# vincenthz/eccoxide

Hardware: AMD Instinct MI355X
Metric: variable-base scalarmuls/sec (batch) per GPU + achieved HBM GB/s vs roofline (higher is better)
Workload: dtype u32

## Files before the change

### __graft_entry__.py

```python
import os
import subprocess
import sys
from concurrent.futures import ThreadPoolExecutor

ROOT = os.path.dirname(os.path.abspath(__file__))
if ROOT not in sys.path:
    sys.path.insert(0, ROOT)


def build() -> None:
    jobs = str(min(6, os.cpu_count() or 1))
    subprocess.check_call(["make", "-C", os.path.join(ROOT, "eccoxide_amd", "csrc"), "-j", jobs, "ARCH=gfx950"])
    subprocess.check_call(["make", "-C", os.path.join(ROOT, "oracle")])
    subprocess.check_call(["make", "-C", os.path.join(ROOT, "tests", "cpp")])
    test_libs = [
        "hip",
        "hip_p256k1",
        "hip_ed25519",
        "hip_merged",
        "hip_signed",
        "hip_lo32",
        "hip_ecdsa",
        "hip_ed25519_sign",
        "hip_ecdsa_sign",
        "hip_h2c",
        "hip_g2",
        "hip_h2c_g2",
        "hip_pairing",
        "hip_x448",
        "hip_jubjub",
        "hip_msm",
        "hip_sat",
    ]
    with ThreadPoolExecutor(max_workers=int(jobs)) as pool:
        list(pool.map(lambda d: subprocess.check_call(["make", "-C", os.path.join(ROOT, "tests", d)]), test_libs))
    import eccoxide_amd
    from eccoxide_amd import _lib

    lib = _lib.load()
    assert lib.eccx_field_bytes(eccoxide_amd.P256R1) == 32


def smoke() -> None:
    import eccoxide_amd as E
    from eccoxide_amd import workload as W
    from tests import oracle_lib

    ora = oracle_lib.load()
    with E.Engine(0) as eng:
        for curve, n in (("p256r1", 300), ("ed25519", 300)):
            ks = W.random_scalars(curve, n, seed=1).tobytes()
            want_b = ora.base(curve, ks, threads=4)
            got_b = eng.scalarmul_base(curve, ks)
            assert got_b[0] == want_b[0] and got_b[1] == want_b[1], f"{curve}: fixed-base mismatch vs oracle"
            pts = want_b[0]
            ks2 = W.random_scalars(curve, n, seed=2).tobytes()
            want_v = ora.var(curve, ks2, pts, threads=4)
            got_d = eng.scalarmul_var(curve, ks2, pts)
            assert got_d[0] == want_v[0] and got_d[1] == want_v[1], f"{curve}: variable-base mismatch vs oracle"
            got_v = eng.scalarmul_var(curve, ks2, pts, want_proj=True)
            assert got_v[0] == want_v[0] and got_v[1] == want_v[1], f"{curve}: mirror variable-base mismatch vs oracle"
            assert got_v[2] == want_v[2], f"{curve}: un-normalised coordinates differ from the reference algorithm"
            for kw in ({"ct_scan": True}, {"ct_gather": True}):
                got_c = eng.scalarmul_base(curve, ks, **kw)
                assert got_c[0] == want_b[0] and got_c[1] == want_b[1], f"{curve} {kw}: secret-scalar fixed base mismatch vs oracle"
            got_c = eng.scalarmul_var(curve, ks2, pts, ct_scan=True)
            assert got_c[0] == want_v[0] and got_c[1] == want_v[1], f"{curve}: secret-scalar variable base mismatch vs oracle"
            from oracle import ecc_ref as R

            inf = None if curve == "ed25519" else got_d[1]
            enc = eng.point_compress(curve, got_d[0], inf)
            assert enc == R.point_compress_bytes(curve, got_d[0], inf), f"{curve}: point encoding differs from the oracle"
            back = eng.point_decompress(curve, enc)
            assert back[0] == got_d[0] and back[1] == (bytes(n) if inf is None else inf), f"{curve}: decompress(compress(P)) != P"
        curve, n = "bls12_381_g1", 200
        pts = ora.base(curve, W.random_scalars(curve, n, seed=3).tobytes(), threads=4)[0]
        ks = W.random_scalars(curve, n, seed=4).tobytes()
        want = ora.var(curve, ks, pts, threads=4)
        for opts in ({}, {"assume_subgroup": True}, {"ct_scan": True}, {"ct_scan": True, "assume_subgroup": True}):
            got = eng.scalarmul_var(curve, ks, pts, **opts)
            assert got[0] == want[0] and got[1] == want[1], f"{curve} {opts}: variable-base mismatch vs oracle"
        from tests import ed25519_ref as ED

        seeds = bytes(range(32)) + bytes(range(32, 64)) + bytes(32)
        msgs = [b"", b"smoke", bytes(200)]
        pubs = eng.ed25519_public_key(seeds)
        assert pubs[:32] == ED.public_key(seeds[:32]), "ed25519: public key differs from the model"
        sigs = eng.ed25519_sign(msgs, seeds)
        assert sigs[64:128] == ED.sign(seeds[32:64], msgs[1]), "ed25519: signature differs from the model"
        assert eng.ed25519_sign(msgs, seeds, pubs) == sigs and eng.ed25519_sign(msgs, seeds, ct_gather=True) == sigs
        assert eng.ed25519_verify(msgs, sigs, pubs) == bytes([E.SIG_VALID]) * 3, "ed25519: own signatures do not verify"
        from tests import ecdsa_ref as EC, ecdsa_sign_ref as ES

        d, k, dig = bytes(range(1, 97)), bytes(range(101, 197)), bytes(range(7, 103))
        keys, kst = eng.ecdsa_public_key("p256r1", d)
        sigs, sst = eng.ecdsa_sign("p256r1", dig, d, k)
        assert (sigs[64:128], sst[1]) == ES.sign_record(EC.CURVES["p256r1"], dig[32:64], d[32:64], k[32:64]), "ecdsa: signature differs from the model"
        assert kst + sst == bytes([E.SIGN_OK]) * 6 and eng.ecdsa_verify("p256r1", dig, sigs, keys) == bytes([E.SIG_VALID]) * 3, "ecdsa: own signatures do not verify"
        from tests import h2c_ref as H2C

        hmsgs, tag = [b"", b"smoke", bytes(200)], b"QUUX-V01-CS02-with-BLS12381G1_XMD:SHA-256_SSWU_RO_"
        assert eng.hash_to_g1(hmsgs, tag) == H2C.hash_records(hmsgs, tag), "bls12_381_g1: hash_to_curve differs from the model"
        assert eng.hash_to_g1(hmsgs, tag, nonuniform=True) == H2C.hash_records(hmsgs, tag, True), \
            "bls12_381_g1: encode_to_curve differs from the model"
        from tests import g2_ref as G2

        n = 24
        rows = W.random_scalars("bls12_381_g2", 2 * n, seed=5)
        ks = [int.from_bytes(r.tobytes(), "big") for r in rows]
        off = G2.point_of_x((1, 2))
        bases = [G2.mul(k, G2.G) for k in ks[n:n + 4]] * (n // 4)
        bases[1], bases[2] = off, G2.add(G2.G, off)
        kb, pb = rows[:n].tobytes(), b"".join(G2.to_record(p)[0] for p in bases)
        want = [G2.to_record(G2.mul(k, p)) for k, p in zip(ks[:n], bases)]
        want = (b"".join(w[0] for w in want), bytes(w[1] for w in want))
        want_b = [G2.to_record(G2.mul(k, G2.G)) for k in ks[:n]]
        want_b = (b"".join(w[0] for w in want_b), bytes(w[1] for w in want_b))
        for ct in (False, True):
# ... 89 lines not shown
```

### eccoxide_amd/csrc/kernels_coz.hpp

```cpp
#pragma once
#include <type_traits>
#include "inv_gcd.hpp"
#include "kernels_ct.hpp"

namespace eccx {

struct NoGlv {
  static constexpr int K_BITS = 0;
};
struct PrimeOrderBases : NoGlv {};

template <class G>
ECCX_DEV void glv_split(uint32_t (&k1)[5], uint32_t (&k2)[5], const uint8_t* __restrict__ kb) {
  uint32_t k[8];
#pragma unroll
  for (int i = 0; i < 8; ++i) {
    const uint8_t* b = kb + 28 - 4 * i;
    k[i] = ((uint32_t)b[0] << 24) | ((uint32_t)b[1] << 16) | ((uint32_t)b[2] << 8) | (uint32_t)b[3];
  }
  uint32_t prod[13];
#pragma unroll
  for (int i = 0; i < 13; ++i) prod[i] = 0;
#pragma unroll
  for (int i = 0; i < 8; ++i) {
// ... 159 lines not shown
  s2 = h2[4] >> 31;
  uint32_t c_1 = s1, c_2 = s2;
#pragma unroll
  for (int i = 0; i < 5; ++i) {
    const uint64_t a = (uint64_t)(h1[i] ^ (0u - s1)) + c_1;
    k1[i] = (uint32_t)a;
    c_1 = (uint32_t)(a >> 32);
    const uint64_t b = (uint64_t)(h2[i] ^ (0u - s2)) + c_2;
    k2[i] = (uint32_t)b;
    c_2 = (uint32_t)(b >> 32);
  }
}


template <class CU>
constexpr int urowc_words() { return ((3 * CU::N + 3) / 4) * 4; }

template <class CU>
ECCX_DEV void u2_load(U<CU, 1, 3>& x, U<CU, 1, 3>& y, const uint32_t* __restrict__ row) {
  constexpr int N = CU::N;
  constexpr int W = ((2 * N + 3) / 4) * 4;
  uint32_t w[W];
  const uint4* src = reinterpret_cast<const uint4*>(row);
#pragma unroll
  for (int i = 0; i < W / 4; ++i) {
    const uint4 q = src[i];
    w[4 * i] = q.x; w[4 * i + 1] = q.y; w[4 * i + 2] = q.z; w[4 * i + 3] = q.w;
  }
#pragma unroll
  for (int i = 0; i < N; ++i) { x.v[i] = w[i]; y.v[i] = w[N + i]; }
}

template <class CU>
constexpr int urow2_words() { return ((2 * CU::N + 3) / 4) * 4; }
#ifndef ECCX_CT_VAR_PK
#define ECCX_CT_VAR_PK 0
#endif
template <class CU, bool TAGGED = false>
ECCX_DEV void u2_store(uint32_t* __restrict__ row, const U<CU, 1, 3>& x, const U<CU, 1, 3>& y) {
  constexpr int N = CU::N;
  constexpr int W = urow2_words<CU>();
  constexpr uint32_t T = TAGGED ? CT_F32_TAG : 0u;
  uint32_t w[W];
#pragma unroll
  for (int i = 0; i < W; ++i) w[i] = (i < N ? x.v[i] : (i < 2 * N ? y.v[i - N] : 0u)) | T;
  uint4* dst = reinterpret_cast<uint4*>(row);
#pragma unroll
  for (int i = 0; i < W / 4; ++i) dst[i] = make_uint4(w[4 * i], w[4 * i + 1], w[4 * i + 2], w[4 * i + 3]);
}

template <class CU>
ECCX_DEV void ujac_madd_signed(UJac<CU>& r, bool& h_zero, bool& r_zero, const UJac<CU>& p,
                          const U<CU, 1, 3>& x2, const U<CU, 1, 3>& y2, bool neg) {
  auto z1z1 = u_sqr(p.z);
  auto u2 = u_mul(x2, z1z1);
  auto t = u_mul(p.z, z1z1);
  U<CU, 2, 4> sy;
  u_select(sy, neg, u_neg(y2), u_as<2, 4>(y2));
  auto s2 = u_mul(u_reduce(sy), t);
  auto h = u_reduce(u_sub(u2, p.x));
  auto rr = u_reduce(u_sub(s2, p.y));
  h_zero = u_is_zero_mod_p(h);
  r_zero = u_is_zero_mod_p(rr);
  auto hh = u_sqr(h);
  auto hhh = u_mul(h, hh);
  auto v = u_mul(p.x, hh);
  auto r2 = u_sqr(rr);
  auto x3 = u_reduce(u_sub(u_sub(u_sub(r2, hhh), v), v));
  r.x = x3;
  if constexpr (CU::KIND == UK_MONT) {
    r.y = u_fit<1, 3>(u_mul_add(rr, u_sub(v, x3), u_neg(p.y), hhh));
  } else if constexpr (UB<CU>::SPARSE) {
    r.y = u_mul_sub(rr, u_sub(v, x3), p.y, hhh);
  } else if constexpr (UBS<CU>::DENSE) {
    r.y = u_mul_sub(rr, u_sdiff(v, x3), p.y, hhh);
  } else {
    auto y3a = u_mul(rr, u_sub(v, x3));
    auto y1h = u_mul(p.y, hhh);
    r.y = u_reduce(u_sub(y3a, y1h));
  }
  r.z = u_fit<UJac<CU>::ZK, UJac<CU>::ZV>(u_mul(p.z, h));
}

template <class CU>
ECCX_DEV void uzaddu(U<CU, 1, 3>& x1, U<CU, 1, 3>& y1, U<CU, 1, 3>& x2, U<CU, 1, 3>& y2, U<CU, 1, 3>& d_out, bool& d_zero) {
  const auto d = u_reduce(u_sub(x1, x2));
  d_zero = u_is_zero_mod_p(d);
  const auto c = u_sqr(d);
  const U<CU, 1, 3> w1 = u_fit<1, 3>(u_mul(x1, c));
  const auto w2 = u_mul(x2, c);
  const auto e = u_reduce(u_sub(y1, y2));
  const auto dd = u_sqr(e);
  const U<CU, 1, 3> a1 = u_fit<1, 3>(u_mul(y1, u_sub(w1, w2)));
  const auto x3 = u_reduce(u_sub(u_sub(dd, w1), w2));
  const auto y3m = u_mul(e, u_sub(w1, x3));
  x2 = x3;
  y2 = u_reduce(u_sub(y3m, a1));
  x1 = w1;
  y1 = a1;
  d_out = d;
}

template <class CU>
ECCX_DEV void ujac_madd_ct(UJac<CU>& r, bool& h_zero, bool& r_zero, const UJac<CU>& p, const U<CU, 1, 3>& x2,
                           const U<CU, 1, 3>& y2) {
  auto z1z1 = u_sqr(p.z);
  auto u2 = u_mul(x2, z1z1);
  auto t = u_mul(p.z, z1z1);
  auto s2 = u_mul(y2, t);
  auto h = u_reduce(u_sub(u2, p.x));
  auto rr = u_reduce(u_sub(s2, p.y));
  h_zero = u_is_zero_mod_p_ct(h);
  r_zero = u_is_zero_mod_p_ct(rr);
  auto hh = u_sqr(h);
  auto hhh = u_mul(h, hh);
  auto v = u_mul(p.x, hh);
  auto r2 = u_sqr(rr);
  auto x3 = u_reduce(u_sub(u_sub(u_sub(r2, hhh), v), v));
  r.x = x3;
  if constexpr (CU::KIND == UK_MONT) {
    r.y = u_fit<1, 3>(u_mul_add(rr, u_sub(v, x3), u_neg(p.y), hhh));
  } else if constexpr (UB<CU>::SPARSE) {
    r.y = u_mul_sub(rr, u_sub(v, x3), p.y, hhh);
  } else {
    auto y3a = u_mul(rr, u_sub(v, x3));
    auto y1h = u_mul(p.y, hhh);
    r.y = u_reduce(u_sub(y3a, y1h));
  }
  r.z = u_fit<UJac<CU>::ZK, UJac<CU>::ZV>(u_mul(p.z, h));
}

template <class CU>
ECCX_DEV void ujac_dbl_affine(U<CU, 1, 3>& x3, U<CU, 1, 3>& y3, U<CU, 1, 3>& z3, U<CU, 1, 3>& sv, U<CU, 1, 3>& y8v,
                              const U<CU, 1, 3>& px, const U<CU, 1, 3>& py) {
  const auto xx = u_sqr(px);
  const auto yy = u_sqr(py);
  const auto yyyy = u_sqr(yy);
  const auto xyy = u_mul(px, yy);
  const auto s2 = u_add(xyy, xyy);
  sv = u_reduce(u_add(s2, s2));
  const auto y4 = u_add(yyyy, yyyy);
  const auto y8 = u_add(y4, y4);
  y8v = u_reduce(u_add(y8, y8));
  if constexpr (CU::Sat::A0 == 1) {
    const auto m = u_reduce(u_add(u_add(xx, xx), xx));
    x3 = u_reduce(u_sub(u_sub(u_sqr(m), sv), sv));
    y3 = u_reduce(u_sub(u_mul(m, u_sub(sv, x3)), y8v));
  } else {
    U<CU, 1, 3> one;
#pragma unroll
    for (int i = 0; i < CU::N; ++i) one.v[i] = CU::ONE[i];
    const auto xm = u_sub(xx, one);
    const auto m = u_reduce(u_add(u_add(xm, xm), xm));
    x3 = u_reduce(u_sub(u_sub(u_sqr(m), sv), sv));
    y3 = u_reduce(u_sub(u_mul(m, u_sub(sv, x3)), y8v));
  }
  z3 = u_reduce(u_add(py, py));
}

template <class CU, int WB, bool ASSUME_PRIME = false>
constexpr int coz_full_windows() {
  using CS = typename CU::Sat;
  constexpr int NWIN = (8 * CS::SB + 1 + WB - 1) / WB;
  return (CS::PRIME_ORDER || ASSUME_PRIME) ? (8 * CS::SB - CS::NBITS + 1) / WB + 1 : NWIN;
}
#ifndef ECCX_CT_VAR_BITS
#define ECCX_CT_VAR_BITS 4
#endif

#ifndef ECCX_COZ_OCC_U14
#define ECCX_COZ_OCC_U14 3
#endif
#ifndef ECCX_COZ_OCC_BLS
#define ECCX_COZ_OCC_BLS 2
#endif
#ifndef ECCX_COZ_OCC_U9
#define ECCX_COZ_OCC_U9 4
#endif
#ifndef ECCX_COZ_NESTED_LADDER
#define ECCX_COZ_NESTED_LADDER 1
#endif
template <class CU, bool GLV>
constexpr int coz_occupancy() {
  return CU::N <= 9 ? ECCX_COZ_OCC_U9
                    : (CU::N <= 14 ? (GLV ? ECCX_OCC_U14 : (CU::KIND == UK_MONT ? ECCX_COZ_OCC_BLS : ECCX_COZ_OCC_U14)) : ECCX_OCC_U18);
}


template <class CU, class G, bool GLV, bool FUSED = false, int WB = 5, bool CT = false>
__global__ void __launch_bounds__(WG, (coz_occupancy<CU, GLV>())) k_scalarmul_coz_unsat(size_t n, const uint8_t* __restrict__ scalars,
                                                                                 const uint8_t* __restrict__ points,
                                                                                 uint32_t* __restrict__ rows_out,
                                                                                 uint8_t* __restrict__ flags,
                                                                                 uint32_t* __restrict__ scratch, uint32_t opts,
                                                                                 const uint8_t* __restrict__ base_scalars = nullptr,
                                                                                 const uint32_t* __restrict__ utable = nullptr) {
  static_assert(!(GLV && FUSED), "the verify shape takes any curve point");
  static_assert(!(CT && FUSED), "the verify shape has no secret-scalar form");
  constexpr bool ASSUME_PRIME = std::is_same<G, PrimeOrderBases>::value;
  constexpr bool LATTICE = GlvLattice<G>::value;
  static_assert(!(LATTICE && CT), "the secret-scalar endomorphism ladder is written for the unsigned split");
  static_assert(!ASSUME_PRIME || CT, "PrimeOrderBases only narrows the secret-scalar form's collision windows");
  static_assert(WB >= 3 && WB <= 5, "table rows 1 .. 2^(WB-1) must fit the slab");
  constexpr int TBL = 1 << (WB - 1);
  using CS = typename CU::Sat;
  constexpr bool ISO = CS::A0 == 1;
  constexpr int L = CS::L;
  constexpr int N = CU::N;
  constexpr int FB = CS::FB;
  constexpr int SB = CS::SB;
  static_assert(!GLV || SB == 32, "the split is written for 256-bit scalars");
  constexpr int NWIN = GLV ? (G::K_BITS + 1 + WB - 1) / WB : (8 * SB + 1 + WB - 1) / WB;
  constexpr int S = (!GLV && !CT) ? (8 * SB + 1) % WB : 0;
  constexpr int NWIN_MAIN = S != 0 ? (8 * SB + 1) / WB : NWIN;
  constexpr bool SHARED_INV = !ISO && !CT;
  static_assert(WG == 256, "the shared inversion multiplies the values of four waves");
  constexpr int WR = urowc_words<CU>();
  static_assert(!ISO || WR >= 16 + N, "row 0 holds the split scalar and zeta");
  using T = U<CU, 1, 3>;
  uint32_t* slab = scratch + ((size_t)blockIdx.x * FAST_TABLE_ROWS * WG + threadIdx.x) * (size_t)WR;
  auto row = [&](uint32_t e) { return slab + (size_t)e * WG * WR; };
  constexpr int WC = urow2_words<CU>();
  static_assert(!CT || (size_t)TBL * WC <= (size_t)(FAST_TABLE_ROWS - 1 - TBL) * WR, "the compact table must fit the free rows");
  uint32_t* cslab = scratch + ((size_t)blockIdx.x * FAST_TABLE_ROWS + (TBL + 1)) * WG * (size_t)WR + (size_t)threadIdx.x * WC;
  auto crow = [&](uint32_t e) { return cslab + (size_t)(e - 1) * WG * WC; };
  uint32_t iter = 0u;
  for (size_t base = (size_t)blockIdx.x * WG; base < n; base += (size_t)gridDim.x * WG, ++iter) {
    const size_t gid = base + threadIdx.x;
    const bool active = gid < n;
    const size_t idx = active ? gid : n - 1;
    const uint8_t* __restrict__ k = scalars + idx * (size_t)SB;
    if constexpr (GLV) {
      uint32_t k1[5], k2[5], s1 = 0, s2 = 0;
      if constexpr (LATTICE) glv_split_lattice<G>(k1, k2, s1, s2, k);
      else glv_split<G>(k1, k2, k);
      uint4* d = reinterpret_cast<uint4*>(row(0));
      d[0] = make_uint4(k1[0], k1[1], k1[2], k1[3]);
      d[1] = make_uint4(k1[4], s1, 0u, 0u);
      d[2] = make_uint4(k2[0], k2[1], k2[2], k2[3]);
      d[3] = make_uint4(k2[4], s2, 0u, 0u);
    }
    const uint32_t* kw = row(0);

    T one;
#pragma unroll
    for (int i = 0; i < N; ++i) one.v[i] = CU::ONE[i];
    UJac<CU> q;
    bool rejected = false;
    {
      Fe<L> rx, ry;
      fe_load_be<CS>(rx, points + idx * (size_t)(2 * FB));
      fe_load_be<CS>(ry, points + idx * (size_t)(2 * FB) + FB);
      if (opts & OPT_VALIDATE) {
        Fe<L> mx, my;
        fe_to_mont<CS>(mx, rx);
        fe_to_mont<CS>(my, ry);
        rejected = !(fe_is_canonical<CS>(rx) && fe_is_canonical<CS>(ry) && on_curve<CS>(mx, my));
      }
      q.x = u_as<1, 3>(u_to_mont<CU>(rx));
      q.y = u_as<1, 3>(u_to_mont<CU>(ry));
    }
    if constexpr (FUSED) {
      if (opts & OPT_NEGATE_B) q.y = u_reduce(u_neg(q.y));
    }
    q.z = u_as<UJac<CU>::ZK, UJac<CU>::ZV>(one);
    u3_store<CU>(row(1), q.x, q.y, one);

    auto booth = [&](int w, bool second, uint32_t& d, bool& neg) {
      uint32_t w6;
      if constexpr (GLV) {
        const uint32_t* h = kw + (second ? 8 : 0);
        const int pos = WB * w - 1 + 32;
        const int wi = pos >> 5, sh = pos & 31;
        const uint32_t lo = (wi >= 1 && wi <= 5) ? h[wi - 1] : 0u;
        const uint32_t hi = (wi <= 4) ? h[wi] : 0u;
        w6 = (uint32_t)((((uint64_t)hi << 32) | lo) >> sh) & ((1u << (WB + 1)) - 1u);
        const uint32_t s = ~((w6 >> WB) - 1u);
        const uint32_t m = (((1u << (WB + 1)) - w6 - 1u) & s) | (w6 & ~s);
        d = (m >> 1) + (m & 1u);
        neg = (s & 1u) != 0;
        if constexpr (LATTICE) neg = neg != (h[5] != 0u);
      } else if constexpr (S != 0) {
        booth_digit_aligned<WB, SB, S>(k, w, d, neg);
      } else {
        booth_digit<WB, SB>(k, w, d, neg);
      }
    };

    bool degenerate = false;
    {
      T px = q.x, py = q.y;
      T tx, ty, ratio;
      T zacc = one;
      {
        T x3, y3, sv, y8v;
        ujac_dbl_affine<CU>(x3, y3, ratio, sv, y8v, px, py);
        degenerate = u_is_zero_mod_p(ratio);
        tx = x3;
        ty = y3;
        px = sv;
        py = y8v;
        if constexpr (!ISO) zacc = ratio;
        u3_store<CU>(row(2), tx, ty, ratio);
      }
      for (int d = 3; d <= TBL; ++d) {
        bool dz;
        uzaddu<CU>(px, py, tx, ty, ratio, dz);
        degenerate = degenerate || dz;
        if constexpr (!ISO) zacc = u_fit<1, 3>(u_mul(zacc, ratio));
        u3_store<CU>(row(d), tx, ty, ratio);
      }
      T lam = one, next = ratio;
      if constexpr (ISO) {
        if constexpr (CT) u2_store<CU, (ECCX_CT_VAR_PK != 0)>(crow(TBL), tx, ty);
        else if constexpr (GLV) u3_store<CU>(row(TBL), tx, ty, u_fit<1, 3>(u_mul_k<CU>(tx, CU::BETA)));
      } else {
        if constexpr (SHARED_INV) {
          __shared__ uint32_t zsh[N][WG];
          const uint32_t tid = threadIdx.x;
          T zs;
          u_select(zs, degenerate, one, zacc);
#pragma unroll
          for (int i = 0; i < N; ++i) zsh[i][tid] = zs.v[i];
          __syncthreads();
          if ((uint32_t)__builtin_amdgcn_readfirstlane((int)(tid >> 6)) == (iter & 3u)) {
            const uint32_t col = tid & 63u;
            auto get = [&](int j) {
              T a;
#pragma unroll
              for (int i = 0; i < N; ++i) a.v[i] = zsh[i][col + 64u * j];
              return a;
            };
            auto put = [&](int j, const T& a) {
#pragma unroll
              for (int i = 0; i < N; ++i) zsh[i][col + 64u * j] = a.v[i];
            };
            const T p1 = u_fit<1, 3>(u_mul(get(0), get(1)));
            const T p2 = u_fit<1, 3>(u_mul(p1, get(2)));
            Fe<L> c;
            u_to_canonical<CU>(c, u_mul(p2, get(3)));
            fe_inv_gcd<CS>(c, c);
            T inv = u_as<1, 3>(u_to_mont<CU>(c));
            {
              const T a3 = get(3);
              put(3, u_fit<1, 3>(u_mul(inv, p2)));
              inv = u_fit<1, 3>(u_mul(inv, a3));
            }
            {
              const T a2 = get(2);
              put(2, u_fit<1, 3>(u_mul(inv, p1)));
              inv = u_fit<1, 3>(u_mul(inv, a2));
            }
            const T a0 = get(0), a1 = get(1);
            put(0, u_fit<1, 3>(u_mul(inv, a1)));
            put(1, u_fit<1, 3>(u_mul(inv, a0)));
          }
          __syncthreads();
#pragma unroll
          for (int i = 0; i < N; ++i) lam.v[i] = zsh[i][tid];
          __syncthreads();
        } else {
          Fe<L> c;
          u_to_canonical<CU>(c, zacc);
          fe_inv_gcd<CS>(c, c);
          lam = u_as<1, 3>(u_to_mont<CU>(c));
        }
        const T l2 = u_fit<1, 3>(u_sqr(lam));
        const T l3 = u_fit<1, 3>(u_mul(l2, lam));
        const T xt = u_fit<1, 3>(u_mul(tx, l2)), yt = u_fit<1, 3>(u_mul(ty, l3));
        if constexpr (CT) u2_store<CU, (ECCX_CT_VAR_PK != 0)>(crow(TBL), xt, yt);
        else u3_store<CU>(row(TBL), xt, yt, one);
      }
      for (int d = TBL - 1; d >= 1; --d) {
        lam = u_fit<1, 3>(u_mul(lam, next));
        T x, y;
        u3_load<CU>(x, y, next, row(d));
        const T l2 = u_fit<1, 3>(u_sqr(lam));
        const T l3 = u_fit<1, 3>(u_mul(l2, lam));
        const T xs = u_fit<1, 3>(u_mul(x, l2));
        const T ys = u_fit<1, 3>(u_mul(y, l3));
        if constexpr (CT) u2_store<CU, (ECCX_CT_VAR_PK != 0)>(crow(d), xs, ys);
        else if constexpr (GLV) u3_store<CU>(row(d), xs, ys, u_fit<1, 3>(u_mul_k<CU>(xs, CU::BETA)));
        else u3_store<CU>(row(d), xs, ys, one);
      }
      if constexpr (ISO) {
        uint32_t* zdst = row(0) + 16;
#pragma unroll
        for (int i = 0; i < N; ++i) zdst[i] = lam.v[i];
      }
    }

    if constexpr (CT) {
      constexpr int FULLW = GLV ? 1 : coz_full_windows<CU, WB, ASSUME_PRIME>();
      constexpr int HALVES = GLV ? 2 : 1;
      auto lookup = [&](int w, bool second, T& ex, T& ey, uint32_t& d) {
        bool neg;
        booth(w, second, d, neg);
        neg = neg != second;
#if ECCX_CT_VAR_PK
        {
          uint64_t acc[N];
#pragma unroll
          for (int p = 0; p < N; ++p) acc[p] = 0;
#pragma unroll 2
          for (int j = 1; j <= TBL; ++j) {
            uint32_t m;
            asm("v_cndmask_b32_e64 %0, 0, 1.0, %1" : "=v"(m) : "s"(__builtin_amdgcn_uicmp(d, (uint32_t)j, 32 )));
            const uint64_t m2 = m;
            const uint4* src = reinterpret_cast<const uint4*>(crow(j));
            uint4 v[WC / 4];
#pragma unroll
            for (int c = 0; c < WC / 4; ++c) v[c] = src[c];
#pragma unroll
            for (int p = 0; p < N; ++p) {
              const uint4 qv = v[p / 2];
              ct_fsel2(acc[p], (p & 1) ? (((uint64_t)qv.w << 32) | qv.z) : (((uint64_t)qv.y << 32) | qv.x), m2);
            }
          }
#pragma unroll
          for (int i = 0; i < N; ++i) {
            ex.v[i] = (uint32_t)(acc[i / 2] >> (32 * (i & 1))) & ~CT_F32_TAG;
            ey.v[i] = (uint32_t)(acc[(N + i) / 2] >> (32 * ((N + i) & 1))) & ~CT_F32_TAG;
          }
        }
#else
        u_set_zero(ex);
        u_set_zero(ey);
#pragma unroll 2
        for (int j = 1; j <= TBL; ++j) {
          T cx, cy;
          u2_load<CU>(cx, cy, crow(j));
          const uint64_t m = __builtin_amdgcn_uicmp(d, (uint32_t)j, 32 );
          u_cmov_ct(ex, m, cx);
          u_cmov_ct(ey, m, cy);
        }
#endif
        if constexpr (GLV) {
          if (second) ex = u_fit<1, 3>(u_mul_k<CU>(ex, CU::BETA));
        }
        U<CU, 2, 4> sy;
        u_select_ct(sy, neg, u_neg(ey), u_as<2, 4>(ey));
        ey = u_reduce(sy);
      };
      T zero;
      u_set_zero(zero);
      using TZ = U<CU, UJac<CU>::ZK, UJac<CU>::ZV>;
      {
        T ex, ey;
        uint32_t d;
        lookup(NWIN - 1, false, ex, ey, d);
        q.x = ex;
        q.y = ey;
        u_select_ct(q.z, d == 0, u_as<UJac<CU>::ZK, UJac<CU>::ZV>(zero), u_as<UJac<CU>::ZK, UJac<CU>::ZV>(one));
      }
#pragma unroll 1
      for (int win = NWIN - 1; win >= 0; --win) {
        if (win != NWIN - 1) {
#pragma unroll 1
          for (int j = 0; j < WB; ++j) {
            UJac<CU> t;
            ujac_dbl<CU>(t, q);
            q = t;
          }
        }
#pragma unroll 1
        for (int half = (win == NWIN - 1) ? 1 : 0; half < HALVES; ++half) {
          T ex, ey;
          uint32_t d;
          lookup(win, half != 0, ex, ey, d);
          const bool q_inf = u_limbs_all_zero(q.z);
          const bool e_skip = d == 0;
          UJac<CU> sum;
          bool hz, rz;
          ujac_madd_ct<CU>(sum, hz, rz, q, ex, ey);
          if (win < FULLW) {
            T dx, dy, dz, sv, y8v;
            ujac_dbl_affine<CU>(dx, dy, dz, sv, y8v, ex, ey);
            const bool same_x = hz & !q_inf & !e_skip;
            const uint64_t mt = ct_mask(same_x & rz);
            const uint64_t mc = ct_mask(same_x & !rz);
            u_cmov_ct(sum.x, mt, dx);
            u_cmov_ct(sum.y, mt, dy);
            u_cmov_ct(sum.z, mt, TZ(u_as<UJac<CU>::ZK, UJac<CU>::ZV>(dz)));
            u_cmov_ct(sum.z, mc, TZ(u_as<UJac<CU>::ZK, UJac<CU>::ZV>(zero)));
          }
          const uint64_t mi = ct_mask(q_inf), mk = ct_mask(!e_skip);
          u_cmov_ct(sum.x, mi, ex);
          u_cmov_ct(sum.y, mi, ey);
          u_cmov_ct(sum.z, mi, TZ(u_as<UJac<CU>::ZK, UJac<CU>::ZV>(one)));
          u_cmov_ct(q.x, mk, sum.x);
          u_cmov_ct(q.y, mk, sum.y);
          u_cmov_ct(q.z, mk, sum.z);
        }
      }
    } else {
      constexpr int WIN_END = S != 0 ? -1 : 0;
      {
        uint32_t d;
        bool neg;
        booth(NWIN_MAIN - 1, false, d, neg);
        T tx, ty;
        u2_load<CU>(tx, ty, row(d ? d : 1));
        U<CU, 2, 4> sy;
        u_select(sy, neg, u_neg(ty), u_as<2, 4>(ty));
        q.x = tx;
        q.y = u_reduce(sy);
        q.z = u_as<UJac<CU>::ZK, UJac<CU>::ZV>(one);
        if (d == 0) u_set_zero(q.z);
      }
      bool fix_lane = false;
      auto dbl_step = [&](bool fix) __attribute__((always_inline)) {
        UJac<CU> t;
        if constexpr (UBS<CU>::DENSE) {
          ujac_dbl_merged<CU>(t, q);
          if (fix) {
            const uint64_t keep = ct_mask(!fix_lane);
            u_cmov_ct(t.x, keep, q.x);
            u_cmov_ct(t.y, keep, q.y);
            u_cmov_ct(t.z, keep, q.z);
          }
          q = t;
        } else {
          ujac_dbl<CU>(t, q);
          if (fix) {
            u_select(q.x, fix_lane, t.x, q.x);
            u_select(q.y, fix_lane, t.y, q.y);
            u_select(q.z, fix_lane, t.z, q.z);
          } else {
            q = t;
          }
        }
      };
      auto add_step = [&](int win, bool second) __attribute__((always_inline)) -> bool {
        uint32_t d;
        bool neg;
        booth(win, second, d, neg);
        if (second && !LATTICE) neg = !neg;
        T ex, ey;
        if constexpr (GLV) {
          T eb;
          u3_load<CU>(ex, ey, eb, row(d ? d : 1));
          if (second) ex = eb;
        } else {
          u2_load<CU>(ex, ey, row(d ? d : 1));
        }
        const bool q_inf = u_limbs_all_zero(q.z);
        const bool e_skip = (d == 0);
        UJac<CU> sum;
        bool hz, rz;
        ujac_madd_signed<CU>(sum, hz, rz, q, ex, ey, neg);
        const bool same_x = hz && !q_inf && !e_skip;
        fix_lane = same_x && rz;
        if (same_x && !rz) u_set_zero(sum.z);
        if (__builtin_amdgcn_ballot_w64(q_inf) != 0) {
          U<CU, 2, 4> sy;
          u_select(sy, neg, u_neg(ey), u_as<2, 4>(ey));
          u_select(sum.x, q_inf, ex, sum.x);
          u_select(sum.y, q_inf, u_reduce(sy), sum.y);
          u_select(sum.z, q_inf, u_as<UJac<CU>::ZK, UJac<CU>::ZV>(one), sum.z);
        }
        const bool keep = e_skip || fix_lane;
        u_select(q.x, keep, q.x, sum.x);
        u_select(q.y, keep, q.y, sum.y);
        u_select(q.z, keep, q.z, sum.z);
        return __builtin_amdgcn_ballot_w64(fix_lane) != 0;
      };
      if constexpr (!GLV && ECCX_COZ_NESTED_LADDER) {
#pragma unroll 1
        for (int win = NWIN_MAIN - 2; win >= WIN_END; --win) {
          const int nd = (S != 0 && win < 0) ? S : WB;
#pragma unroll 1
          for (int sub = 0; sub < nd; ++sub) dbl_step(false);
          if (add_step(win, false)) dbl_step(true);
        }
      } else {
        int win, sub;
        if constexpr (GLV) {
          win = NWIN_MAIN - 1;
          sub = WB + 1;
        } else {
          win = NWIN_MAIN - 2;
          sub = 0;
        }
        bool fix_pending = false;
        while (win >= WIN_END) {
          const int nd = (S != 0 && win < 0) ? S : WB;
          bool step_done;
          if (fix_pending || sub < nd) {
            dbl_step(fix_pending);
            fix_pending = false;
            step_done = true;
          } else {
            fix_pending = add_step(win, GLV && sub == WB + 1);
            step_done = !fix_pending;
          }
          if (step_done) {
            if (sub < nd + (GLV ? 1 : 0)) {
              ++sub;
            } else {
              sub = 0;
              --win;
            }
          }
        }
      }
    }
    if constexpr (ISO) {
      T zeta;
      const uint32_t* zsrc = row(0) + 16;
#pragma unroll
      for (int i = 0; i < N; ++i) zeta.v[i] = zsrc[i];
      q.z = u_fit<UJac<CU>::ZK, UJac<CU>::ZV>(u_mul(q.z, zeta));
    }
    if constexpr (FUSED) ucomb_accumulate<CU, false>(q, base_scalars + idx * (size_t)SB, utable);
    if (active) {
      u3_store<CU>(rows_out + idx * (size_t)urow3_words<CU>(), q.x, q.y, u_fit<1, 3>(q.z));
      flags[idx] = rejected ? 2 : (degenerate ? FLAG_REDO : 0);
    }
  }
}

}
```

### eccoxide_amd/csrc/ufe.hpp

```cpp
#pragma once
#include "fe.hpp"

#include <type_traits>

#ifndef ECCX_SOLINAS_REDUCE
#define ECCX_SOLINAS_REDUCE 1
#endif

namespace eccx {

#include "umad_chunks.inc"

__device__ __forceinline__ void smad1_k(uint64_t& acc, uint32_t a, int32_t k) {
  asm("v_mad_i64_i32 %0, vcc, %1, %2, %0" : "+v"(acc) : "v"(a), "s"(k) : "vcc");
}

__device__ __forceinline__ void smad1_v(uint64_t& acc, int32_t a, int32_t b) {
  asm("v_mad_i64_i32 %0, vcc, %1, %2, %0" : "+v"(acc) : "v"(a), "v"(b) : "vcc");
}

template <int S>
__device__ __forceinline__ void ucarry_hi(uint64_t& acc) {
  uint64_t r;
  asm("v_mad_u64_u32 %0, vcc, %1, %2, 0" : "=&v"(r) : "v"((uint32_t)(acc >> 32)), "n"(1 << S) : "vcc");
// ... 789 lines not shown
  u_mul2_core_mont<C>(r.v, a.v, b.v, c.v, d.v);
  return r;
}

template <class C>
struct UBS {
  static constexpr bool OK = UB<C>::SPARSE || C::KIND == UK_MONT;
  static constexpr bool DENSE = C::KIND == UK_MONT_PP1 && !UB<C>::SPARSE;
  static constexpr int KKS = (int)((~(uint64_t)0 >> 1) / ((uint64_t)C::N * UB<C>::COL)) - 1;
  static_assert(!DENSE || (uint64_t)C::N * KKS * UB<C>::COL <= (~(uint64_t)0 >> 1) - 0xffffffffull * UB<C>::pp1_sum() -
                                                                ((uint64_t)1 << C::B) - ((uint64_t)1 << (63 - C::B)),
                "32-bit Montgomery digits overflow the signed columns");
  static constexpr bool ks_ok(int k) { return ((uint64_t)(k + 1) << C::B) <= ((uint64_t)1 << 31); }
};

template <class C, int K1, int V1, int K2, int V2, int K3, int V3, int K4, int V4>
ECCX_DEV auto u_mul_sub(const U<C, K1, V1>& a, const U<C, K2, V2>& b, const U<C, K3, V3>& c, const U<C, K4, V4>& d) {
  static_assert(UBS<C>::OK || UBS<C>::DENSE, "implemented for the Montgomery fields with room for signed columns");
  static_assert(K1 * K2 <= UBS<C>::KKS && K3 * K4 <= UBS<C>::KKS, "a product overflows the signed columns");
  static_assert(UBS<C>::ks_ok(K3) && UBS<C>::ks_ok(K4), "negated / signed operands must stay below 2^31");
  static_assert((uint32_t)(V1 * V2) < C::RP && (uint32_t)(V3 * V4) < C::RP, "result outside (0, 3p)");
  U<C, 1, 3> r;
  if constexpr (UB<C>::SPARSE) u_mul_sub_core_sparse<C, false>(r.v, a.v, b.v, c.v, d.v);
  else if constexpr (UBS<C>::DENSE) u_mul_sub_core_pp1<C, false>(r.v, a.v, b.v, c.v, d.v);
  else u_mul_sub_core_mont<C, false>(r.v, a.v, b.v, c.v, d.v);
  return r;
}
template <class C, int K1, int V1, int K2, int V2, int K3, int V3>
ECCX_DEV auto u_mul_sub_2sqr(const U<C, K1, V1>& a, const U<C, K2, V2>& b, const U<C, K3, V3>& c) {
  static_assert(UBS<C>::OK || UBS<C>::DENSE, "implemented for the Montgomery fields with room for signed columns");
  static_assert(K1 * K2 <= UBS<C>::KKS && 2 * K3 * K3 <= UBS<C>::KKS, "a product overflows the signed columns");
  static_assert(UBS<C>::ks_ok(2 * K3), "doubled / negated operands must stay below 2^31");
  static_assert((uint32_t)(V1 * V2) < C::RP && (uint32_t)(2 * V3 * V3) < C::RP, "result outside (0, 3p)");
  U<C, 1, 3> r;
  if constexpr (UB<C>::SPARSE) u_mul_sub_core_sparse<C, true>(r.v, a.v, b.v, c.v, c.v);
  else if constexpr (UBS<C>::DENSE) u_mul_sub_core_pp1<C, true>(r.v, a.v, b.v, c.v, c.v);
  else u_mul_sub_core_mont<C, true>(r.v, a.v, b.v, c.v, c.v);
  return r;
}

template <class C, int K, int V>
struct US {
  static_assert(K >= 1 && UBS<C>::ks_ok(K), "signed limbs must stay below 2^31");
  static_assert(V >= 1 && V <= 4096, "value bound out of range");
  int32_t v[C::N];
};

template <class C, int V1, int V2>
ECCX_DEV auto u_sdiff(const U<C, 1, V1>& a, const U<C, 1, V2>& b) {
  US<C, 1, (V1 > V2 ? V1 : V2)> r;
#pragma unroll
  for (int i = 0; i < C::N; ++i) r.v[i] = (int32_t)(a.v[i] - b.v[i]);
  return r;
}

template <class C>
constexpr bool ubs_neg_side_ok(int kk) {
  return (uint64_t)C::N * (uint64_t)kk * UB<C>::COL <= (~(uint64_t)0 >> 1) - ((uint64_t)1 << (64 - C::B));
}

template <class C, int K1, int V1, int K2, int V2, int K3, int V3, int K4, int V4>
ECCX_DEV auto u_mul_sub(const U<C, K1, V1>& a, const US<C, K2, V2>& b, const U<C, K3, V3>& c, const U<C, K4, V4>& d) {
  static_assert(UBS<C>::DENSE, "signed operands are implemented for p = -1 mod 2^B with p + 1 as plain digits");
  static_assert(K1 * K2 <= UBS<C>::KKS && K3 * K4 <= UBS<C>::KKS, "a product overflows the signed columns");
  static_assert(UBS<C>::ks_ok(K1) && UBS<C>::ks_ok(K3) && UBS<C>::ks_ok(K4), "negated / signed operands must stay below 2^31");
  static_assert(ubs_neg_side_ok<C>(K1 * K2 + K3 * K4), "the negative side of a column overflows");
  static_assert((uint32_t)(V1 * V2 + V3 * V4) < C::RP, "result outside (0, 3p)");
  U<C, 1, 3> r;
  u_mul_sub_core_pp1<C, false, int32_t>(r.v, a.v, b.v, c.v, d.v);
  return r;
}
template <class C, int K1, int V1, int K2, int V2, int K3, int V3>
ECCX_DEV auto u_mul_sub_2sqr(const U<C, K1, V1>& a, const US<C, K2, V2>& b, const U<C, K3, V3>& c) {
  static_assert(UBS<C>::DENSE, "signed operands are implemented for p = -1 mod 2^B with p + 1 as plain digits");
  static_assert(K1 * K2 <= UBS<C>::KKS && 2 * K3 * K3 <= UBS<C>::KKS, "a product overflows the signed columns");
  static_assert(UBS<C>::ks_ok(K1) && UBS<C>::ks_ok(2 * K3), "doubled / negated operands must stay below 2^31");
  static_assert(ubs_neg_side_ok<C>(K1 * K2 + 2 * K3 * K3), "the negative side of a column overflows");
  static_assert((uint32_t)(V1 * V2 + 2 * V3 * V3) < C::RP, "result outside (0, 3p)");
  U<C, 1, 3> r;
  u_mul_sub_core_pp1<C, true, int32_t>(r.v, a.v, b.v, c.v, c.v);
  return r;
}

template <class C, int V1>
ECCX_DEV auto u_sqr2(const U<C, 1, V1>& a) {
  static_assert(UBS<C>::DENSE && UB<C>::LO32, "written for p = -1 mod 2^B with p + 1 as plain digits");
  static_assert(UB<C>::kk_ok(2, 1), "columns: a square with doubled terms carries a product with K1*K2 = 2");
  static_assert(UB<C>::KMAX >= 2, "limbs: the doubled operand a << 1 (below 2 * 2^B) stays below 2^32");
  static_assert(UB<C>::vout(2 * V1, V1) <= 3, "result too large: reduce the operand first");
  U<C, 1, UB<C>::vout(2 * V1, V1)> r;
  u_mul_core_mont<C, true, false, true, true>(r.v, a.v, a.v);
  return r;
}

template <class C, int K1, int V1>
ECCX_DEV auto u_sqr(const U<C, K1, V1>& a) {
  if constexpr (!UB<C>::ksq_ok(K1) || (UB<C>::vout(V1, V1) > 3)) {
    return u_sqr(u_reduce(a));
  } else {
    U<C, 1, UB<C>::vout(V1, V1)> r;
    u_mul_core<C, true, false>(r.v, a.v, a.v);
    return r;
  }
}

template <class C, int K1, int V1>
ECCX_DEV auto u_mul_k(const U<C, K1, V1>& a, const uint32_t (&k)[C::N]) {
  if constexpr (!UB<C>::kk_ok(K1, 1) || (UB<C>::vout(V1, 1) > 3)) {
    return u_mul_k(u_reduce(a), k);
  } else {
    U<C, 1, UB<C>::vout(V1, 1)> r;
    u_mul_core<C, false, true>(r.v, a.v, k);
    return r;
  }
}

template <class C>
ECCX_DEV U<C, 1, 2> u_mul_k_exit(const U<C, 1, 3>& a, const uint32_t (&k)[C::N]) {
  static_assert(UB<C>::MONT && UB<C>::vout(3, 1) <= 2, "Montgomery fields; a reduced operand times a constant below p");
  U<C, 1, 2> r;
  u_mul_core_mont<C, false, true, false>(r.v, a.v, k);
  return r;
}

template <class C, int K1, int V1>
ECCX_DEV U<C, 1, 2> u_mul_small(const U<C, K1, V1>& a, uint32_t k) {
  static_assert(C::KIND == UK_PM19 || C::KIND == UK_GOLDILOCKS, "written for 2^255 - 19 and 2^448 - 2^224 - 1");
  constexpr int N = C::N;
  uint32_t t[N];
  uint64_t acc = 0;
#pragma unroll
  for (int i = 0; i < N; ++i) {
    umad1_v(acc, a.v[i], k);
    t[i] = (uint32_t)acc & C::MASK;
    acc >>= C::B;
  }
  if constexpr (C::KIND == UK_GOLDILOCKS) u_gold_tail<C>(t, acc);
  else u_pm_tail<C>(t, acc);
  U<C, 1, 2> r;
#pragma unroll
  for (int i = 0; i < N; ++i) r.v[i] = t[i];
  return r;
}

template <class C, int K1, int V1, int K2, int V2>
ECCX_DEV auto u_add(const U<C, K1, V1>& a, const U<C, K2, V2>& b) {
  if constexpr (K1 + K2 > UB<C>::KMAX) {
    if constexpr (K1 >= K2) return u_add(u_reduce(a), b);
    else return u_add(a, u_reduce(b));
  } else {
    U<C, K1 + K2, V1 + V2> r;
#pragma unroll
    for (int i = 0; i < C::N; ++i) r.v[i] = a.v[i] + b.v[i];
    return r;
  }
}

template <class C, int K1, int V1, int K2, int V2>
ECCX_DEV auto u_sub(const U<C, K1, V1>& a, const U<C, K2, V2>& b) {
  if constexpr (K2 != 1 || V2 > 3) {
    return u_sub(a, u_reduce(b));
  } else if constexpr (K1 + 2 > UB<C>::KMAX) {
    return u_sub(u_reduce(a), b);
  } else {
    U<C, K1 + 2, V1 + 4> r;
#pragma unroll
// ... 179 lines not shown
```

Measured before the change: 79.09 million.

## Use signed-difference madd and precomputed negated-y table entries in COZ ladder

For public-scalar, non-GLV curves with dense p = -1 mod 2^B, the mixed add now forms H and R as signed differences. It squares and multiplies them with new signed Montgomery kernels, which skips the reductions, and does the zero tests only on wave-uniform rare paths through Z3. The precomputed table also stores -y in its third slot, so the Booth digit sign picks a column at load time instead of negating and reducing each step. A signed co-Z addition for table building is added but left off by default, and a standalone signed-square check build is added to the setup.

```diff
diff --git a/__graft_entry__.py b/__graft_entry__.py
--- a/__graft_entry__.py
+++ b/__graft_entry__.py
@@ -32,8 +32,10 @@
         "hip_msm",
         "hip_sat",
     ]
+    makes = [["make", "-C", os.path.join(ROOT, "tests", d)] for d in test_libs]
+    makes.append(["make", "-C", os.path.join(ROOT, "tests", "hip"), "-f", "signed_sq_check.mk"])
     with ThreadPoolExecutor(max_workers=int(jobs)) as pool:
-        list(pool.map(lambda d: subprocess.check_call(["make", "-C", os.path.join(ROOT, "tests", d)]), test_libs))
+        list(pool.map(subprocess.check_call, makes))
     import eccoxide_amd
     from eccoxide_amd import _lib
 
diff --git a/eccoxide_amd/csrc/kernels_coz.hpp b/eccoxide_amd/csrc/kernels_coz.hpp
--- a/eccoxide_amd/csrc/kernels_coz.hpp
+++ b/eccoxide_amd/csrc/kernels_coz.hpp
@@ -265,6 +265,76 @@
   r.z = u_fit<UJac<CU>::ZK, UJac<CU>::ZV>(u_mul(p.z, h));
 }
 
+#ifndef ECCX_COZ_MADD_SIGNED_HR
+#define ECCX_COZ_MADD_SIGNED_HR 1
+#endif
+#ifndef ECCX_COZ_TABLE_NEG_Y
+#define ECCX_COZ_TABLE_NEG_Y 1
+#endif
+#ifndef ECCX_COZ_ZADDU_SIGNED
+#define ECCX_COZ_ZADDU_SIGNED 0
+#endif
+
+template <class CU>
+ECCX_DEV void u2_load_xc(U<CU, 1, 3>& x, U<CU, 1, 3>& y, const uint32_t* __restrict__ row, bool third) {
+  constexpr int N = CU::N;
+  const uint32_t* xs = static_cast<const uint32_t*>(__builtin_assume_aligned(row, 16));
+  const uint32_t* ys = row + (third ? 2 * N : N);
+#pragma unroll
+  for (int i = 0; i < N; ++i) x.v[i] = xs[i];
+#pragma unroll
+  for (int i = 0; i < N; ++i) y.v[i] = ys[i];
+}
+
+template <class CU>
+ECCX_DEV void ujac_madd_shr(UJac<CU>& r, bool& z3_zero, US<CU, 1, 3>& h_out, US<CU, 1, 3>& r_out, const UJac<CU>& p,
+                            const U<CU, 1, 3>& x2, const U<CU, 1, 3>& y2) {
+  static_assert(UBS<CU>::DENSE, "written for p = -1 mod 2^B with p + 1 as plain digits");
+  auto z1z1 = u_sqr(p.z);
+  auto u2 = u_mul(x2, z1z1);
+  auto t = u_mul(p.z, z1z1);
+  auto s2 = u_mul(y2, t);
+  const auto h = u_sdiff(u2, p.x);
+  const auto rr = u_sdiff(s2, p.y);
+  auto hh = u_ssqr(h);
+  auto hhh = u_smul(hh, h);
+  auto v = u_mul(p.x, hh);
+  auto r2 = u_ssqr(rr);
+  auto x3 = u_reduce(u_sub(u_sub(u_sub(r2, hhh), v), v));
+  r.x = x3;
+  r.y = u_mul_sub(rr, u_sdiff(v, x3), p.y, hhh);
+  const U<CU, 1, 3> z3 = u_smul(p.z, h);
+  z3_zero = u_is_zero_mod_p(z3);
+  r.z = u_as<UJac<CU>::ZK, UJac<CU>::ZV>(z3);
+  h_out = h;
+  r_out = rr;
+}
+
+template <class CU>
+ECCX_DEV void ujac_madd_ys(UJac<CU>& r, bool& h_zero, bool& r_zero, const UJac<CU>& p, const U<CU, 1, 3>& x2,
+                           const U<CU, 1, 3>& y2) {
+  static_assert(UBS<CU>::DENSE, "written for p = -1 mod 2^B with p + 1 as plain digits");
+  auto z1z1 = u_sqr(p.z);
+  auto u2 = u_mul(x2, z1z1);
+  auto t = u_mul(p.z, z1z1);
+  auto s2 = u_mul(y2, t);
+  auto h = u_reduce(u_sub(u2, p.x));
+  auto rr = u_reduce(u_sub(s2, p.y));
+  h_zero = u_is_zero_mod_p(h);
+  r_zero = u_is_zero_mod_p(rr);
+  auto hh = u_sqr(h);
+  auto hhh = u_mul(h, hh);
+  auto v = u_mul(p.x, hh);
+  auto r2 = u_sqr(rr);
+  auto x3 = u_reduce(u_sub(u_sub(u_sub(r2, hhh), v), v));
+  r.x = x3;
+  r.y = u_mul_sub(rr, u_sdiff(v, x3), p.y, hhh);
+  r.z = u_fit<UJac<CU>::ZK, UJac<CU>::ZV>(u_mul(p.z, h));
+}
+
+template <class CU>
+ECCX_DEV bool us_is_zero_mod_p(const US<CU, 1, 3>& a) { return u_is_zero_mod_p(u_reduce(u_unsigned(a))); }
+
 template <class CU>
 ECCX_DEV void uzaddu(U<CU, 1, 3>& x1, U<CU, 1, 3>& y1, U<CU, 1, 3>& x2, U<CU, 1, 3>& y2, U<CU, 1, 3>& d_out, bool& d_zero) {
   const auto d = u_reduce(u_sub(x1, x2));
@@ -282,6 +352,51 @@
   x1 = w1;
   y1 = a1;
   d_out = d;
+}
+
+template <class CU>
+ECCX_DEV void uzaddu_signed(U<CU, 1, 3>& x1, U<CU, 1, 3>& y1, U<CU, 1, 3>& x2, U<CU, 1, 3>& y2, US<CU, 1, 3>& d_out) {
+  static_assert(UBS<CU>::DENSE, "written for p = -1 mod 2^B with p + 1 as plain digits");
+  const auto d = u_sdiff(x1, x2);
+  const auto c = u_ssqr(d);
+  const U<CU, 1, 3> w1 = u_fit<1, 3>(u_mul(x1, c));
+  const auto w2 = u_mul(x2, c);
+  const auto e = u_sdiff(y1, y2);
+  const auto dd = u_ssqr(e);
+  const U<CU, 1, 3> a1 = u_fit<1, 3>(u_mul(y1, u_sub(w1, w2)));
+  const auto x3 = u_reduce(u_sub(u_sub(dd, w1), w2));
+  const auto y3m = u_smul(e, u_sdiff(w1, x3));
+  x2 = x3;
+  y2 = u_reduce(u_sub(y3m, a1));
+  x1 = w1;
+  y1 = a1;
+  d_out = d;
+}
+
+template <class CU>
+ECCX_DEV void u3_store(uint32_t* __restrict__ row, const U<CU, 1, 3>& x, const U<CU, 1, 3>& y, const US<CU, 1, 3>& z) {
+  constexpr int N = CU::N;
+  constexpr int W = urow3_words<CU>();
+  uint32_t w[W];
+#pragma unroll
+  for (int i = 0; i < W; ++i) w[i] = i < N ? x.v[i] : (i < 2 * N ? y.v[i - N] : (i < 3 * N ? (uint32_t)z.v[i - 2 * N] : 0u));
+  uint4* dst = reinterpret_cast<uint4*>(row);
+#pragma unroll
+  for (int i = 0; i < W / 4; ++i) dst[i] = make_uint4(w[4 * i], w[4 * i + 1], w[4 * i + 2], w[4 * i + 3]);
+}
+template <class CU>
+ECCX_DEV void u3_load(U<CU, 1, 3>& x, U<CU, 1, 3>& y, US<CU, 1, 3>& z, const uint32_t* __restrict__ row) {
+  constexpr int N = CU::N;
+  constexpr int W = urow3_words<CU>();
+  uint32_t w[W];
+  const uint4* src = reinterpret_cast<const uint4*>(row);
+#pragma unroll
+  for (int i = 0; i < W / 4; ++i) {
+    const uint4 q = src[i];
+    w[4 * i] = q.x; w[4 * i + 1] = q.y; w[4 * i + 2] = q.z; w[4 * i + 3] = q.w;
+  }
+#pragma unroll
+  for (int i = 0; i < N; ++i) { x.v[i] = w[i]; y.v[i] = w[N + i]; z.v[i] = (int32_t)w[2 * N + i]; }
 }
 
 template <class CU>
@@ -401,6 +516,12 @@
   constexpr int WR = urowc_words<CU>();
   static_assert(!ISO || WR >= 16 + N, "row 0 holds the split scalar and zeta");
   using T = U<CU, 1, 3>;
+  constexpr bool DENSE_PUB = UBS<CU>::DENSE && !CT && !GLV;
+  constexpr bool MADD_SHR = DENSE_PUB && ECCX_COZ_MADD_SIGNED_HR != 0;
+  constexpr bool NEG_Y = DENSE_PUB && ECCX_COZ_TABLE_NEG_Y != 0;
+  constexpr bool ZADDU_S = DENSE_PUB && ECCX_COZ_ZADDU_SIGNED != 0;
+  static_assert(!ZADDU_S || !ISO, "the signed ratios' product is the a = -3 ladders' zeta");
+  using TR = std::conditional_t<ZADDU_S, US<CU, 1, 3>, T>;
   uint32_t* slab = scratch + ((size_t)blockIdx.x * FAST_TABLE_ROWS * WG + threadIdx.x) * (size_t)WR;
   auto row = [&](uint32_t e) { return slab + (size_t)e * WG * WR; };
   constexpr int WC = urow2_words<CU>();
@@ -473,27 +594,37 @@
     bool degenerate = false;
     {
       T px = q.x, py = q.y;
-      T tx, ty, ratio;
+      T tx, ty;
+      TR ratio;
       T zacc = one;
       {
-        T x3, y3, sv, y8v;
-        ujac_dbl_affine<CU>(x3, y3, ratio, sv, y8v, px, py);
-        degenerate = u_is_zero_mod_p(ratio);
+        T x3, y3, z2, sv, y8v;
+        ujac_dbl_affine<CU>(x3, y3, z2, sv, y8v, px, py);
+        if constexpr (!ZADDU_S) degenerate = u_is_zero_mod_p(z2);
         tx = x3;
         ty = y3;
         px = sv;
         py = y8v;
-        if constexpr (!ISO) zacc = ratio;
+        if constexpr (!ISO) zacc = z2;
+        if constexpr (ZADDU_S) ratio = u_signed(z2);
+        else ratio = z2;
         u3_store<CU>(row(2), tx, ty, ratio);
       }
       for (int d = 3; d <= TBL; ++d) {
-        bool dz;
-        uzaddu<CU>(px, py, tx, ty, ratio, dz);
-        degenerate = degenerate || dz;
-        if constexpr (!ISO) zacc = u_fit<1, 3>(u_mul(zacc, ratio));
+        if constexpr (ZADDU_S) {
+          uzaddu_signed<CU>(px, py, tx, ty, ratio);
+          zacc = u_smul(zacc, ratio);
+        } else {
+          bool dz;
+          uzaddu<CU>(px, py, tx, ty, ratio, dz);
+          degenerate = degenerate || dz;
+          if constexpr (!ISO) zacc = u_fit<1, 3>(u_mul(zacc, ratio));
+        }
         u3_store<CU>(row(d), tx, ty, ratio);
       }
-      T lam = one, next = ratio;
+      if constexpr (ZADDU_S) degenerate = u_is_zero_mod_p(zacc);
+      T lam = one;
+      TR next = ratio;
       if constexpr (ISO) {
         if constexpr (CT) u2_store<CU, (ECCX_CT_VAR_PK != 0)>(crow(TBL), tx, ty);
         else if constexpr (GLV) u3_store<CU>(row(TBL), tx, ty, u_fit<1, 3>(u_mul_k<CU>(tx, CU::BETA)));
@@ -552,10 +683,12 @@
         const T l3 = u_fit<1, 3>(u_mul(l2, lam));
         const T xt = u_fit<1, 3>(u_mul(tx, l2)), yt = u_fit<1, 3>(u_mul(ty, l3));
         if constexpr (CT) u2_store<CU, (ECCX_CT_VAR_PK != 0)>(crow(TBL), xt, yt);
+        else if constexpr (NEG_Y) u3_store<CU>(row(TBL), xt, yt, u_reduce(u_neg(yt)));
         else u3_store<CU>(row(TBL), xt, yt, one);
       }
       for (int d = TBL - 1; d >= 1; --d) {
-        lam = u_fit<1, 3>(u_mul(lam, next));
+        if constexpr (ZADDU_S) lam = u_smul(lam, next);
+        else lam = u_fit<1, 3>(u_mul(lam, next));
         T x, y;
         u3_load<CU>(x, y, next, row(d));
         const T l2 = u_fit<1, 3>(u_sqr(lam));
@@ -564,6 +697,7 @@
         const T ys = u_fit<1, 3>(u_mul(y, l3));
         if constexpr (CT) u2_store<CU, (ECCX_CT_VAR_PK != 0)>(crow(d), xs, ys);
         else if constexpr (GLV) u3_store<CU>(row(d), xs, ys, u_fit<1, 3>(u_mul_k<CU>(xs, CU::BETA)));
+        else if constexpr (NEG_Y) u3_store<CU>(row(d), xs, ys, u_reduce(u_neg(ys)));
         else u3_store<CU>(row(d), xs, ys, one);
       }
       if constexpr (ISO) {
@@ -683,11 +817,16 @@
         bool neg;
         booth(NWIN_MAIN - 1, false, d, neg);
         T tx, ty;
-        u2_load<CU>(tx, ty, row(d ? d : 1));
-        U<CU, 2, 4> sy;
-        u_select(sy, neg, u_neg(ty), u_as<2, 4>(ty));
+        if constexpr (NEG_Y) {
+          u2_load_xc<CU>(tx, ty, row(d ? d : 1), neg);
+          q.y = ty;
+        } else {
+          u2_load<CU>(tx, ty, row(d ? d : 1));
+          U<CU, 2, 4> sy;
+          u_select(sy, neg, u_neg(ty), u_as<2, 4>(ty));
+          q.y = u_reduce(sy);
+        }
         q.x = tx;
-        q.y = u_reduce(sy);
         q.z = u_as<UJac<CU>::ZK, UJac<CU>::ZV>(one);
         if (d == 0) u_set_zero(q.z);
       }
@@ -724,23 +863,57 @@
           T eb;
           u3_load<CU>(ex, ey, eb, row(d ? d : 1));
           if (second) ex = eb;
-        } else {
+        } else if constexpr (!NEG_Y) {
           u2_load<CU>(ex, ey, row(d ? d : 1));
         }
         const bool q_inf = u_limbs_all_zero(q.z);
         const bool e_skip = (d == 0);
         UJac<CU> sum;
-        bool hz, rz;
-        ujac_madd_signed<CU>(sum, hz, rz, q, ex, ey, neg);
-        const bool same_x = hz && !q_inf && !e_skip;
-        fix_lane = same_x && rz;
-        if (same_x && !rz) u_set_zero(sum.z);
-        if (__builtin_amdgcn_ballot_w64(q_inf) != 0) {
-          U<CU, 2, 4> sy;
-          u_select(sy, neg, u_neg(ey), u_as<2, 4>(ey));
-          u_select(sum.x, q_inf, ex, sum.x);
-          u_select(sum.y, q_inf, u_reduce(sy), sum.y);
-          u_select(sum.z, q_inf, u_as<UJac<CU>::ZK, UJac<CU>::ZV>(one), sum.z);
+        if constexpr (MADD_SHR || NEG_Y) {
+          if constexpr (NEG_Y) {
+            u2_load_xc<CU>(ex, ey, row(d ? d : 1), neg);
+          } else {
+            U<CU, 2, 4> sy;
+            u_select(sy, neg, u_neg(ey), u_as<2, 4>(ey));
+            ey = u_reduce(sy);
+          }
+          if constexpr (MADD_SHR) {
+            US<CU, 1, 3> h, rr;
+            bool zz;
+            ujac_madd_shr<CU>(sum, zz, h, rr, q, ex, ey);
+            const bool maybe_same_x = zz && !q_inf && !e_skip;
+            fix_lane = false;
+            if (__builtin_amdgcn_ballot_w64(maybe_same_x) != 0) {
+              const bool same_x = maybe_same_x && us_is_zero_mod_p<CU>(h);
+              const bool rz = us_is_zero_mod_p<CU>(rr);
+              fix_lane = same_x && rz;
+              if (same_x && !rz) u_set_zero(sum.z);
+            }
+          } else {
+            bool hz, rz;
+            ujac_madd_ys<CU>(sum, hz, rz, q, ex, ey);
+            const bool same_x = hz && !q_inf && !e_skip;
+            fix_lane = same_x && rz;
+            if (same_x && !rz) u_set_zero(sum.z);
+          }
+          if (__builtin_amdgcn_ballot_w64(q_inf) != 0) {
+            u_select(sum.x, q_inf, ex, sum.x);
+            u_select(sum.y, q_inf, ey, sum.y);
+            u_select(sum.z, q_inf, u_as<UJac<CU>::ZK, UJac<CU>::ZV>(one), sum.z);
+          }
+        } else {
+          bool hz, rz;
+          ujac_madd_signed<CU>(sum, hz, rz, q, ex, ey, neg);
+          const bool same_x = hz && !q_inf && !e_skip;
+          fix_lane = same_x && rz;
+          if (same_x && !rz) u_set_zero(sum.z);
+          if (__builtin_amdgcn_ballot_w64(q_inf) != 0) {
+            U<CU, 2, 4> sy;
+            u_select(sy, neg, u_neg(ey), u_as<2, 4>(ey));
+            u_select(sum.x, q_inf, ex, sum.x);
+            u_select(sum.y, q_inf, u_reduce(sy), sum.y);
+            u_select(sum.z, q_inf, u_as<UJac<CU>::ZK, UJac<CU>::ZV>(one), sum.z);
+          }
         }
         const bool keep = e_skip || fix_lane;
         u_select(q.x, keep, q.x, sum.x);
diff --git a/eccoxide_amd/csrc/ufe.hpp b/eccoxide_amd/csrc/ufe.hpp
--- a/eccoxide_amd/csrc/ufe.hpp
+++ b/eccoxide_amd/csrc/ufe.hpp
@@ -895,6 +895,109 @@
   return r;
 }
 
+template <class C, int K1, int V1, int K2, int V2, int K3, int V3, int K4, int V4>
+ECCX_DEV auto u_mul_sub(const US<C, K1, V1>& a, const US<C, K2, V2>& b, const U<C, K3, V3>& c, const U<C, K4, V4>& d) {
+  static_assert(UBS<C>::DENSE, "signed operands are implemented for p = -1 mod 2^B with p + 1 as plain digits");
+  static_assert(K1 * K2 <= UBS<C>::KKS && K3 * K4 <= UBS<C>::KKS, "a product overflows the signed columns");
+  static_assert(UBS<C>::ks_ok(K3) && UBS<C>::ks_ok(K4), "negated / signed operands must stay below 2^31");
+  static_assert(ubs_neg_side_ok<C>(K1 * K2 + K3 * K4), "the negative side of a column overflows");
+  static_assert((uint32_t)(V1 * V2 + V3 * V4) < C::RP, "result outside (0, 3p)");
+  uint32_t aw[C::N];
+#pragma unroll
+  for (int i = 0; i < C::N; ++i) aw[i] = (uint32_t)a.v[i];
+  U<C, 1, 3> r;
+  u_mul_sub_core_pp1<C, false, int32_t>(r.v, aw, b.v, c.v, d.v);
+  return r;
+}
+
+template <class C, bool SQR>
+ECCX_DEV void u_smul_core_pp1(uint32_t (&r)[C::N], const int32_t (&a)[C::N], const int32_t (&b)[C::N]) {
+  constexpr int N = C::N;
+  static_assert(C::KIND == UK_MONT_PP1 && C::SPARSE_N == 0, "p = -1 mod 2^B with p + 1 as plain digits");
+  uint32_t m[N], t[N];
+  int32_t a2[N];
+  if constexpr (SQR) {
+#pragma unroll
+    for (int i = 0; i < N; ++i) a2[i] = a[i] * 2;
+  }
+  uint64_t acc = 0;
+  UMacQS<32 - C::B> qa;
+  UMacQ<true> qm;
+#pragma unroll
+  for (int k = 0; k < 2 * N - 1; ++k) {
+    const int lo = k < N ? 0 : k - N + 1, hi = k < N ? k : N - 1;
+    if (k >= N && C::P[k - N] != 0) acc += (uint64_t)C::P[k - N];
+    if constexpr (SQR) {
+#pragma unroll
+      for (int i = lo; 2 * i < k; ++i) qa.push(acc, (uint32_t)a[i], a2[k - i]);
+      if ((k & 1) == 0) qa.push(acc, (uint32_t)a[k / 2], a[k / 2]);
+    } else {
+#pragma unroll
+      for (int i = lo; i <= hi; ++i) qa.push(acc, (uint32_t)a[i], b[k - i]);
+    }
+    qa.flush(acc);
+#pragma unroll
+    for (int i = lo; i <= (k < N ? k - 1 : N - 1); ++i) {
+      if (C::PP1[k - i] != 0) qm.push(acc, m[i], C::PP1[k - i]);
+    }
+    qm.flush(acc);
+    if (k < N - 1) {
+      m[k] = (uint32_t)acc;
+      qa.carry(acc);
+      continue;
+    }
+    if (k < N) m[k] = (uint32_t)acc & C::MASK;
+    else t[k - N] = (uint32_t)acc & C::MASK;
+    acc = (uint64_t)((int64_t)acc >> C::B);
+  }
+  acc += (uint64_t)C::P[N - 1];
+  t[N - 1] = (uint32_t)acc;
+#pragma unroll
+  for (int i = 0; i < N; ++i) r[i] = t[i];
+}
+
+template <class C, int K, int V>
+ECCX_DEV US<C, K, V> u_signed(const U<C, K, V>& a) {
+  US<C, K, V> r;
+#pragma unroll
+  for (int i = 0; i < C::N; ++i) r.v[i] = (int32_t)a.v[i];
+  return r;
+}
+
+template <class C, int V>
+ECCX_DEV U<C, 3, V + 4> u_unsigned(const US<C, 1, V>& a) {
+  U<C, 3, V + 4> r;
+#pragma unroll
+  for (int i = 0; i < C::N; ++i) r.v[i] = C::BIAS[i] + (uint32_t)a.v[i];
+  return r;
+}
+
+template <class C, int K1, int V1, int K2, int V2>
+ECCX_DEV U<C, 1, 3> u_smul(const US<C, K1, V1>& a, const US<C, K2, V2>& b) {
+  static_assert(UBS<C>::DENSE && UB<C>::LO32, "signed operands are implemented for p = -1 mod 2^B with p + 1 as plain digits");
+  static_assert(K1 * K2 <= UBS<C>::KKS, "the product overflows the signed columns");
+  static_assert(ubs_neg_side_ok<C>(K1 * K2), "the negative side of a column overflows");
+  static_assert((uint32_t)(V1 * V2) < C::RP, "result outside (0, 3p)");
+  U<C, 1, 3> r;
+  u_smul_core_pp1<C, false>(r.v, a.v, b.v);
+  return r;
+}
+template <class C, int K1, int V1, int K2, int V2>
+ECCX_DEV U<C, 1, 3> u_smul(const U<C, K1, V1>& a, const US<C, K2, V2>& b) {
+  static_assert(UBS<C>::ks_ok(K1), "an operand read as signed must stay below 2^31");
+  return u_smul(u_signed(a), b);
+}
+template <class C, int K1, int V1>
+ECCX_DEV U<C, 1, 3> u_ssqr(const US<C, K1, V1>& a) {
+  static_assert(UBS<C>::DENSE && UB<C>::LO32, "signed operands are implemented for p = -1 mod 2^B with p + 1 as plain digits");
+  static_assert(K1 * K1 <= UBS<C>::KKS && UBS<C>::ks_ok(2 * K1), "the square overflows the signed columns or its doubled limbs 2^31");
+  static_assert(ubs_neg_side_ok<C>(K1 * K1), "the negative side of a column overflows");
+  static_assert((uint32_t)(V1 * V1) < C::RP, "result outside (0, 3p)");
+  U<C, 1, 3> r;
+  u_smul_core_pp1<C, true>(r.v, a.v, a.v);
+  return r;
+}
+
 template <class C, int V1>
 ECCX_DEV auto u_sqr2(const U<C, 1, V1>& a) {
   static_assert(UBS<C>::DENSE && UB<C>::LO32, "written for p = -1 mod 2^B with p + 1 as plain digits");
```

Measured after the change: 74.52 million. 5.8% lower.
